# dangvansam/viet-asr

Hardware: AMD Instinct MI355X
Metric: real_time_factor (higher is better)
Workload: dtype f32 via 2xf16 split operands (22-bit significands, 3 f16 MFMA products per multiply, fp32 accumulate); 1 GPU; BASELINE configs[2]: quartznet15x5 greedy CTC, batch=64x10s 16kHz mono per GPU, wav in HBM -> collapsed ids; batch_per_gpu=64, parallelism=utterance-shard x1

## Files before the change

include/vasr_devtools.h:

```cpp
#ifndef VASR_DEVTOOLS_H_
#define VASR_DEVTOOLS_H_
#include "vasr.h"
#ifdef __cplusplus
extern "C" {
#endif

VASR_API int vasr_profile_bracket_overhead(vasr_stream stream, int n, double* out_us);
VASR_API int vasr_fused_tile_choice(int64_t tiles128, int compute_units);
VASR_API int vasr_fused_waves_choice(int kernel, int dual, int tile_cols);
VASR_API int vasr_plan_buffers(vasr_handle* h, int batch, int64_t samples, int64_t mel_frames, int32_t* out, int cap);
VASR_API int vasr_resample_form(double ratio, int nwin, int num_table, int* p, int* q);
VASR_API int vasr_bench_depthwise(const float* d_x, const float* d_w, const int32_t* d_lens, int batch, int channels,
                         int64_t frames, int kernel, float* d_y, vasr_stream stream);
VASR_API int vasr_bench_depthwise_layer(const float* d_x, const float* d_w, const int32_t* d_lens_in, const int32_t* d_lens_out,
                               int batch, int channels, int64_t frames_in, int kernel, int stride, int dilation, float* d_y,
                               uint32_t* d_amax, int amax_stride, vasr_stream stream);
VASR_API int vasr_depthwise_mfma_table_size(int kernel, int dilation);
VASR_API int vasr_pack_depthwise_taps(const float* h_w, int channels, int kernel, int dilation, uint32_t* h_table, float* h_inv);
VASR_API int vasr_bench_depthwise_mfma(const float* d_x, const uint32_t* d_taps, const float* d_tap_inv, const int32_t* d_lens,
                              int batch, int channels, int64_t frames, int kernel, int dilation, float* d_y,
                              uint32_t* d_amax, int amax_stride, vasr_stream stream);
VASR_API int vasr_pack_pointwise(const float* h_w, int cout, int cin, int m_pad, float* h_out);
VASR_API int vasr_conv_gemm_weights(const float* h_w, int cout, int cin, int kernel, float* h_out);
VASR_API int vasr_bench_pointwise(const float* d_x, const float* d_wt, const float* d_scale, const float* d_shift,
                         int batch, int cin, int cout, int64_t frames, float* d_y, vasr_stream stream);

VASR_API int vasr_bench_mfma_sustained(int gemm_mode, int workgroups, int steps, float* d_sink, double* flops, vasr_stream stream);

VASR_API int vasr_pack_pointwise_f16x2(const float* h_w, int cout, int cin, int m_pad, uint16_t* h_out, float* inv_scale);
VASR_API int vasr_bench_pointwise_f16x2(const float* d_x, const uint16_t* d_w16, float w_inv_scale, const float* d_scale,
                               const float* d_shift, int batch, int cin, int cout, int64_t frames, float* d_y,
                               uint32_t* d_amax, int amax_stride, vasr_stream stream);

VASR_API int vasr_pack_pointwise_bf16x3(const float* h_w, int cout, int cin, int m_pad, uint16_t* h_out);
VASR_API int vasr_bench_pointwise_bf16x3(const float* d_x, const uint16_t* d_w3, const float* d_scale, const float* d_shift,
                                int batch, int cin, int cout, int64_t frames, float* d_y, vasr_stream stream);

VASR_API int vasr_bench_groupnorm(const float* d_x, const int32_t* d_lens, int batch, int channels, int64_t frames,
                                  int norm_groups, int shuffle, const float* h_gamma, const float* h_beta, int relu, float* d_y,
                                  vasr_stream stream);
VASR_API int vasr_bench_ctc_head(const float* d_logits, int batch, int64_t frames, int num_classes, float* d_logp,
                                 int64_t* d_pred, vasr_stream stream);
// ... 5 lines not shown
```

viet-asr_amd/_lib.py:

```python
import ctypes as C
import os

import numpy as np
import torch

_HERE = os.path.dirname(os.path.abspath(__file__))
LIB_PATH = os.environ.get("VASR_LIB_PATH") or os.path.join(_HERE, "lib", "libvasr_hip.so")
DEV_LIB_PATH = os.environ.get("VASR_LIB_PATH") or os.path.join(_HERE, "lib", "libvasr_hip_dev.so")


class VasrError(RuntimeError):
    pass


class BlockDesc(C.Structure):
    _fields_ = [(n, C.c_int32) for n in
                ("filters", "repeat", "kernel", "stride", "dilation", "residual", "separable", "residual_dense")]


class FrontendDesc(C.Structure):
    _fields_ = [("sample_rate", C.c_int32), ("n_fft", C.c_int32), ("win_length", C.c_int32),
                ("hop_length", C.c_int32), ("n_mels", C.c_int32), ("preemph", C.c_float),
                ("log_guard", C.c_float), ("normalize", C.c_int32),
                ("h_window", C.POINTER(C.c_float)), ("h_filterbank", C.POINTER(C.c_float)),
# ... 71 lines not shown
    "vasr_classify_f32": (C.c_int, [_P, _P, _P, C.c_int, C.c_int64, C.c_int64, _P, C.c_int, _P, _P, _P, C.c_size_t, _P]),
    "vasr_beam_workspace_bytes": (C.c_size_t, [C.c_int, C.c_int64]),
    "vasr_beam_search_f32": (C.c_int, [_P, C.c_int, C.c_int64, C.c_int, C.c_int, C.c_int, C.c_float, C.c_float, _P,
                                       _P, _P, _P, _P, C.c_size_t, _P]),
    "vasr_beam_search_rows_f32": (C.c_int, [_P, _P, C.c_int, C.c_int64, C.c_int, C.c_int, C.c_int, C.c_float, C.c_float,
                                            _P, _P, _P, _P, _P, C.c_size_t, _P]),
    "vasr_beam_search_nbest_f32": (C.c_int, [_P, _P, C.c_int, C.c_int64, C.c_int, C.c_int, C.c_int, C.c_int, C.c_float,
                                             C.c_float, _P, _P, _P, _P, _P, _P, _P, C.c_size_t, _P]),
    "vasr_lm_create": (C.c_int, [_P, C.c_int, _P, C.c_int, _P, C.c_int, C.c_int, C.c_int, C.c_int, C.c_int, C.c_float,
                                 C.c_float, C.c_float, C.POINTER(_P)]),
    "vasr_lm_destroy": (None, [_P]),
    "vasr_beam_workgroups": (C.c_int, [C.c_int]),
    "vasr_beam_hash_init": (C.c_uint64, []),
    "vasr_beam_hash_step": (C.c_uint64, [C.c_uint64, C.c_uint64]),
    "vasr_last_error": (C.c_char_p, []),
    "vasr_version": (C.c_char_p, []),
    "vasr_abi_version": (C.c_int, []),
    "vasr_algorithmic_work": (C.c_int, [_P, C.c_int, C.c_int64, C.POINTER(C.c_double)]),
    "vasr_profile_begin": (C.c_int, [_P]),
    "vasr_profile_end": (C.c_int, [_P, C.POINTER(C.c_double), C.POINTER(C.c_int64), C.POINTER(C.c_double), C.POINTER(C.c_double)]),
    "vasr_padded_frames": (C.c_int64, [C.c_int64]),
}

DEV_SIGNATURES = {
    "vasr_pack_pointwise_f16x2": (C.c_int, [_P, C.c_int, C.c_int, C.c_int, _P, C.POINTER(C.c_float)]),
    "vasr_bench_pointwise_f16x2": (C.c_int, [_P, _P, C.c_float, _P, _P, C.c_int, C.c_int, C.c_int, C.c_int64, _P, _P,
                                             C.c_int, _P]),
    "vasr_depthwise_mfma_table_size": (C.c_int, [C.c_int, C.c_int]),
    "vasr_pack_depthwise_taps": (C.c_int, [_P, C.c_int, C.c_int, C.c_int, _P, _P]),
    "vasr_bench_depthwise_mfma": (C.c_int, [_P, _P, _P, _P, C.c_int, C.c_int, C.c_int64, C.c_int, C.c_int, _P, _P, C.c_int, _P]),
    "vasr_profile_bracket_overhead": (C.c_int, [_P, C.c_int, C.POINTER(C.c_double)]),
    "vasr_fused_tile_choice": (C.c_int, [C.c_int64, C.c_int]),
    "vasr_fused_waves_choice": (C.c_int, [C.c_int, C.c_int, C.c_int]),
    "vasr_plan_buffers": (C.c_int, [_P, C.c_int, C.c_int64, C.c_int64, C.POINTER(C.c_int32), C.c_int]),
    "vasr_resample_form": (C.c_int, [C.c_double, C.c_int, C.c_int, C.POINTER(C.c_int), C.POINTER(C.c_int)]),
    "vasr_pack_pointwise": (C.c_int, [_P, C.c_int, C.c_int, C.c_int, _P]),
    "vasr_conv_gemm_weights": (C.c_int, [_P, C.c_int, C.c_int, C.c_int, _P]),
    "vasr_pack_pointwise_bf16x3": (C.c_int, [_P, C.c_int, C.c_int, C.c_int, _P]),
    "vasr_bench_pointwise_bf16x3": (C.c_int, [_P, _P, _P, _P, C.c_int, C.c_int, C.c_int, C.c_int64, _P, _P]),
    "vasr_bench_mfma_sustained": (C.c_int, [C.c_int, C.c_int, C.c_int, _P, C.POINTER(C.c_double), _P]),
    "vasr_bench_depthwise": (C.c_int, [_P, _P, _P, C.c_int, C.c_int, C.c_int64, C.c_int, _P, _P]),
    "vasr_bench_depthwise_layer": (C.c_int, [_P, _P, _P, _P, C.c_int, C.c_int, C.c_int64, C.c_int, C.c_int, C.c_int, _P, _P,
                                             C.c_int, _P]),
    "vasr_bench_pointwise": (C.c_int, [_P, _P, _P, _P, C.c_int, C.c_int, C.c_int, C.c_int64, _P, _P]),
    "vasr_bench_groupnorm": (C.c_int, [_P, _P, C.c_int, C.c_int, C.c_int64, C.c_int, C.c_int, _P, _P, C.c_int, _P, _P]),
    "vasr_bench_ctc_head": (C.c_int, [_P, C.c_int, C.c_int64, C.c_int, _P, _P, _P]),
}

ABI_VERSION = 8

_lib = None
_dev = None


def _load(path, tables):
    if not os.path.exists(path):
        raise VasrError(
            f"{path} is missing: build it with `python -c 'import __graft_entry__ as g; g.build()'` "
            "(or `make -C viet-asr_amd/csrc`). There is no CPU fallback for this path.")
    l = C.CDLL(path)
    for table, required in tables:
        for name, (res, args) in table.items():
            fn = getattr(l, name, None)
            if fn is None:
                if required:
                    raise VasrError(f"{path} does not export {name}")
# ... 163 lines not shown
```

viet-asr_amd/csrc/frontend.hip:

```cpp
#include <atomic>

#include "vasr_internal.h"
#include "len_chain.h"
#include "vasr_device.h"

namespace vasr {

namespace {

constexpr int kWaves = 8;
constexpr int kThreads = 64 * kWaves;
constexpr int kNfft = 512;

struct cf { float re, im; };
__device__ __forceinline__ cf cadd(cf a, cf b) { return {a.re + b.re, a.im + b.im}; }
__device__ __forceinline__ cf csub(cf a, cf b) { return {a.re - b.re, a.im - b.im}; }
__device__ __forceinline__ cf cmul(cf a, cf b) { return {a.re * b.re - a.im * b.im, a.re * b.im + a.im * b.re}; }
__device__ __forceinline__ cf cmul_negi(cf a) { return {a.im, -a.re}; }


__device__ __forceinline__ float sample_f32(const float* x, int64_t n) { return x[n]; }
__device__ __forceinline__ float sample_f32(const short* x, int64_t n) { return (float)x[n] * 0x1p-15f; }

template <int kFramesPerBlock, typename S>
// ... 129 lines not shown
  for (int o = 32; o > 0; o >>= 1) v += __shfl_xor(v, o, 64);
  return v;
}

__device__ __forceinline__ int64_t seq_of(int64_t len, int hop) { return (int64_t)ceilf((float)len / (float)hop); }

constexpr int kRowsPerWg = 4;
__device__ __forceinline__ void normalize_row(float* __restrict__ x, int n, int frames, int normalize, double* red) {
  const int tid = threadIdx.x & 255, lane = tid & 63, wv = tid >> 6;
  float mean = 0.f, stdv = 1.f;
  if (normalize) {
    double s = 0.0;
    for (int t = tid; t < n; t += 256) s += (double)x[t];
    s = wave_sum(s);
    if (lane == 0) red[wv] = s;
    __syncthreads();
    const double mu = (((red[0] + red[1]) + red[2]) + red[3]) / (double)n;
    double q = 0.0;
    for (int t = tid; t < n; t += 256) { const double d = (double)x[t] - mu; q += d * d; }
    q = wave_sum(q);
    if (lane == 0) red[4 + wv] = q;
    __syncthreads();
    mean = (float)mu;
    stdv = (float)sqrt((((red[4] + red[5]) + red[6]) + red[7]) / (double)(n - 1));
    stdv = stdv + 1e-5f;
  }
  for (int t = tid; t < frames; t += 256) {
    float v = 0.f;
    if (t < n) v = normalize ? (x[t] - mean) / stdv : x[t];
    x[t] = v;
  }
}

__global__ __launch_bounds__(256 * kRowsPerWg) void normalize_kernel(float* __restrict__ mel, int64_t ld,
                                                                     const int64_t* __restrict__ seq, int rows, int n_mels,
                                                                     int frames, int normalize) {
  __shared__ double red[kRowsPerWg][8];
  const int grp = threadIdx.x >> 8;
  const int row = min((int)blockIdx.x * kRowsPerWg + grp, rows - 1);
  const int64_t n64 = seq[row / n_mels];
  normalize_row(mel + (int64_t)row * ld, (int)(n64 < 0 ? 0 : (n64 > frames ? frames : n64)), frames, normalize, red[grp]);
}

__global__ __launch_bounds__(256) void normalize_all_kernel(float* __restrict__ mel, int64_t ld, const int64_t* __restrict__ seq,
                                                            int n_mels, int frames) {
  __shared__ double red[8];
  const int tid = threadIdx.x, lane = tid & 63, wv = tid >> 6;
  float* x = mel + (int64_t)blockIdx.x * n_mels * ld;
  const int64_t n64 = seq[blockIdx.x];
  const int n = (int)(n64 < 0 ? 0 : (n64 > frames ? frames : n64));
  const double cnt = (double)n * (double)n_mels;
  double s = 0.0;
  for (int f = 0; f < n_mels; ++f)
    for (int t = tid; t < n; t += 256) s += (double)x[(int64_t)f * ld + t];
  s = wave_sum(s);
  if (lane == 0) red[wv] = s;
  __syncthreads();
  const double mu = (((red[0] + red[1]) + red[2]) + red[3]) / cnt;
  double q = 0.0;
  for (int f = 0; f < n_mels; ++f)
    for (int t = tid; t < n; t += 256) { const double d = (double)x[(int64_t)f * ld + t] - mu; q += d * d; }
  q = wave_sum(q);
  if (lane == 0) red[4 + wv] = q;
  __syncthreads();
  const float mean = (float)mu;
  const float stdv = (float)sqrt((((red[4] + red[5]) + red[6]) + red[7]) / (cnt - 1.0)) + 1e-5f;
  for (int f = 0; f < n_mels; ++f)
    for (int t = tid; t < n; t += 256) x[(int64_t)f * ld + t] = (x[(int64_t)f * ld + t] - mean) / stdv;
}

__global__ __launch_bounds__(256 * kRowsPerWg) void normalize_chain_kernel(float* __restrict__ mel, int64_t ld,
                                                              const int64_t* __restrict__ len, int hop, int batch, int n_mels,
                                                              int frames, int normalize, int64_t* __restrict__ seq,
                                                              const LenStep* __restrict__ steps, int n_steps,
                                                              int32_t* __restrict__ lens_tab, float* __restrict__ enc_len,
                                                              const int64_t* __restrict__ wav_len, int frames_cap) {
  __shared__ double red[kRowsPerWg][8];
  const int rows = batch * n_mels, row_wgs = (rows + kRowsPerWg - 1) / kRowsPerWg;
  if ((int)blockIdx.x < row_wgs) {
    const int grp = threadIdx.x >> 8;
    const int row = min((int)blockIdx.x * kRowsPerWg + grp, rows - 1);
    const int64_t n64 = seq_of(len[row / n_mels], hop);
    normalize_row(mel + (int64_t)row * ld, (int)(n64 < 0 ? 0 : (n64 > frames ? frames : n64)), frames, normalize, red[grp]);
    return;
  }
  const int b = ((int)blockIdx.x - row_wgs) * 256 * kRowsPerWg + (int)threadIdx.x;
  const int64_t l0 = b < batch ? seq_of(len[b], hop) : 0;
  if (b < batch) seq[b] = l0;
  len_chain_body(b, l0, batch, steps, n_steps, lens_tab, enc_len, wav_len, hop, frames_cap);
}

}

void launch_stft_logmel(const FrontendTables& tb, const void* wav, bool pcm16, int batch, int64_t samples,
                        const int64_t* row_len, int hop, float preemph, float log_guard, float* mel, int64_t mel_ld, int frames,
                        hipStream_t st) {
  auto go = [&](auto kern, auto* wav, int fpb) {
    const int seg_len = (fpb - 1) * hop + kNfft;
    const size_t lds = (size_t)((seg_len + 3) & ~3) * 4 + kWaves * 256 * 8 + kWaves * (260 + kMelTaps) * 4 + 64 * (fpb + 1) * 4;
    dim3 grid((frames + fpb - 1) / fpb, batch);
    hipLaunchKernelGGL(kern, grid, dim3(kThreads), lds, st, tb, wav, samples, row_len, hop, preemph, log_guard, mel, mel_ld,
                       frames);
  };
  const bool small = (int64_t)((frames + 31) / 32) * batch < 128;
  if (pcm16) {
    if (small) go(stft_logmel_kernel<8, short>, static_cast<const short*>(wav), 8);
    else go(stft_logmel_kernel<32, short>, static_cast<const short*>(wav), 32);
  } else {
    if (small) go(stft_logmel_kernel<8, float>, static_cast<const float*>(wav), 8);
    else go(stft_logmel_kernel<32, float>, static_cast<const float*>(wav), 32);
  }
}

void launch_seq_len(const int64_t* len, int batch, int hop, int64_t* seq, hipStream_t st) {
  hipLaunchKernelGGL(seq_len_kernel, dim3((batch + 63) / 64), dim3(64), 0, st, len, batch, hop, seq);
}

constexpr int kAloneLds = 152 * 1024;

void launch_normalize_all(float* mel, int64_t mel_ld, const int64_t* seq, int batch, int n_mels, int frames, hipStream_t st) {
  static std::atomic<uint64_t> opted{0};
  (void)dyn_lds_opt_in(reinterpret_cast<const void*>(normalize_all_kernel), kAloneLds, opted);
  hipLaunchKernelGGL(normalize_all_kernel, dim3(batch), dim3(256), kAloneLds, st, mel, mel_ld, seq, n_mels, frames);
}

void launch_normalize(float* mel, int64_t mel_ld, const int64_t* seq, int batch, int n_mels, int frames,
                      int normalize, hipStream_t st) {
  const int rows = batch * n_mels;
  static std::atomic<uint64_t> opted{0};
  (void)dyn_lds_opt_in(reinterpret_cast<const void*>(normalize_kernel), kAloneLds, opted);
  hipLaunchKernelGGL(normalize_kernel, dim3((rows + kRowsPerWg - 1) / kRowsPerWg), dim3(256 * kRowsPerWg), normalize ? kAloneLds : 0, st, mel, mel_ld,
                     seq, rows, n_mels, frames, normalize);
}

void launch_normalize_chain(float* mel, int64_t mel_ld, const int64_t* len, int hop, int batch, int n_mels, int frames,
                            int normalize, int64_t* seq, const LenStep* d_steps, int n_steps, int32_t* lens_tab,
                            float* enc_len, const int64_t* wav_len, int frames_cap, hipStream_t st) {
  const int rows = batch * n_mels;
  static std::atomic<uint64_t> opted{0};
  (void)dyn_lds_opt_in(reinterpret_cast<const void*>(normalize_chain_kernel), kAloneLds, opted);
  const int wg = 256 * kRowsPerWg;
  hipLaunchKernelGGL(normalize_chain_kernel, dim3((rows + kRowsPerWg - 1) / kRowsPerWg + (batch + wg - 1) / wg), dim3(wg), normalize ? kAloneLds : 0, st, mel, mel_ld, len, hop, batch,
                     n_mels, frames, normalize, seq, d_steps, n_steps, lens_tab, enc_len, wav_len, frames_cap);
}

}
```

viet-asr_amd/csrc/vasr_api.cpp:

```cpp
#include <hip/hip_runtime.h>

#include <algorithm>
#include <cmath>
#include <cstdarg>
#include <cstdio>
#include <cstring>
#include <memory>
#include <string>

#include "vasr_model.h"

using namespace vasr;

namespace {
thread_local std::string g_err;
}

namespace vasr {

thread_local LaunchProbe g_probe;

int fail(int code, const char* fmt, ...) {
  char buf[512];
  va_list ap;
// ... 173 lines not shown
  if (h->has_encoder && (rc = build_encoder(h))) return rc;
  if (h->has_decoder && (rc = build_decoder(h))) return rc;
  if (h->has_classifier && (rc = build_classifier(h))) return rc;
  HIP_TRY(hipDeviceSynchronize());
  {
    int dev = 0, n = 0;
    if (hipGetDevice(&dev) == hipSuccess && hipDeviceGetAttribute(&n, hipDeviceAttributeMultiprocessorCount, dev) == hipSuccess && n > 0)
      h->n_cu = n;
  }
  h->weights.clear();
  h->finalized = true;
  return 0;
}

int64_t vasr_mel_frames(const vasr_handle* h, int64_t samples) {
  const int hop = (h && h->has_frontend) ? h->fe.hop_length : 160;
  return 1 + samples / hop;
}

int64_t vasr_encoded_frames(const vasr_handle* h, int64_t mel_frames) {
  if (!h || !h->has_encoder || !h->finalized) return mel_frames;
  return enc_frames(h, mel_frames);
}

static size_t sliced_workspace_bytes(const vasr_handle* h, int batch, int64_t T);

static int check_reflect(const vasr_handle* h, int64_t samples) {
  if (samples <= h->fe.n_fft / 2)
    return fail(VASR_ERR_INVALID, "reflect padding needs more than n_fft/2 = %d samples (got %lld)",
                h->fe.n_fft / 2, (long long)samples);
  return 0;
}

static void run_frontend(vasr_handle* h, const float* d_wav, const int64_t* d_len, int batch, int64_t samples, float* mel,
                         int64_t ld, int T, int64_t* seq, hipStream_t st) {
  launch_seq_len(d_len, batch, h->fe.hop_length, seq, st);
  launch_stft_logmel(h->ft, d_wav, false, batch, samples, h->row_independent ? d_len : nullptr, h->fe.hop_length,
                     h->fe.preemph, h->fe.log_guard, mel, ld, T, st);
  launch_normalize(mel, ld, seq, batch, h->fe.n_mels, T, h->fe.normalize == 1, st);
  if (h->fe.normalize == 2) launch_normalize_all(mel, ld, seq, batch, h->fe.n_mels, T, st);
}

size_t vasr_workspace_bytes(const vasr_handle* h, int batch, int64_t samples, int64_t mel_frames) {
  if (!h || !h->finalized || batch <= 0) return 0;
  const int64_t T = samples > 0 ? vasr_mel_frames(h, samples) : mel_frames;
  const size_t whole = plan_ws(h, batch, T).total;
  if (samples > 0 && h->has_frontend && h->has_encoder && h->has_decoder)
    return std::max(whole, sliced_workspace_bytes(h, batch, T));
  return whole;
}

int vasr_melspec_f32(vasr_handle* h, const float* d_wav, const int64_t* d_len, int batch, int64_t samples,
                     float* d_mel, int64_t* d_seq, vasr_stream stream) {
  if (!h || !h->has_frontend || !h->finalized) return fail(VASR_ERR_STATE, "no finalized front end in this handle");
  if (batch <= 0 || !d_wav || !d_len || !d_mel || !d_seq) return fail(VASR_ERR_INVALID, "bad argument");
  if (int rc = check_reflect(h, samples)) return rc;
  hipStream_t st = static_cast<hipStream_t>(stream);
  const int T = (int)vasr_mel_frames(h, samples);
  run_frontend(h, d_wav, d_len, batch, samples, d_mel, T, T, d_seq, st);
  return check_launch("melspec");
}

int vasr_encoder_f32(vasr_handle* h, const float* d_mel, const int64_t* d_seq, int batch, int64_t mel_frames,
                     float* d_enc, float* d_enc_len, void* d_ws, size_t ws_bytes, vasr_stream stream) {
  if (!h || !h->has_encoder || !h->finalized) return fail(VASR_ERR_STATE, "no finalized encoder in this handle");
  if (batch <= 0 || mel_frames <= 0 || !d_mel || !d_seq || !d_enc || !d_ws) return fail(VASR_ERR_INVALID, "bad argument");
  const WsPlan p = plan_ws(h, batch, mel_frames);
  if (ws_bytes < p.total) return fail(VASR_ERR_WORKSPACE, "workspace %zu < %zu bytes", ws_bytes, p.total);
  hipStream_t st = static_cast<hipStream_t>(stream);
  char* ws = static_cast<char*>(d_ws);
  if (port_input_in_place(h))
    return run_encoder(h, d_mel, mel_frames, mel_frames, d_seq, batch, d_enc, p.T1, d_enc_len, ws, p, st);
  float* melp = reinterpret_cast<float*>(ws + p.melp);
  launch_repad(d_mel, mel_frames, batch * h->feat_in, (int)mel_frames, melp, p.Tp0, st);
  return run_encoder(h, melp, p.Tp0, mel_frames, d_seq, batch, d_enc, p.T1, d_enc_len, ws, p, st);
}

int vasr_decoder_logsoftmax_f32(vasr_handle* h, const float* d_enc, int batch, int64_t enc_frames_, float* d_logp,
                                void* d_ws, size_t ws_bytes, vasr_stream stream) {
  if (!h || !h->has_decoder || !h->finalized) return fail(VASR_ERR_STATE, "no finalized decoder in this handle");
  if (batch <= 0 || enc_frames_ <= 0 || !d_enc || !d_logp || !d_ws) return fail(VASR_ERR_INVALID, "bad argument");
  const int64_t ld = pad_frames(enc_frames_);
  const size_t enc_bytes = align_up((size_t)batch * h->dec_feat_in * ld * 4, 256);
  const size_t need_bytes = enc_bytes + (size_t)batch * h->num_classes * ld * 4;
  if (ws_bytes < need_bytes) return fail(VASR_ERR_WORKSPACE, "workspace %zu < %zu bytes", ws_bytes, need_bytes);
  hipStream_t st = static_cast<hipStream_t>(stream);
  float* encp = static_cast<float*>(d_ws);
  float* logits = reinterpret_cast<float*>(static_cast<char*>(d_ws) + enc_bytes);
  launch_repad(d_enc, enc_frames_, batch * h->dec_feat_in, (int)enc_frames_, encp, ld, st);
  AmaxTab ax{};
  const size_t amax_off = align_up(need_bytes, 256), amax_bytes = (size_t)batch * 256 * 4;
  if (h->gemm_mode == 3 && ws_bytes >= amax_off + amax_bytes) {
    ax = AmaxTab{reinterpret_cast<unsigned int*>(static_cast<char*>(d_ws) + amax_off), 256, 0};
    launch_amax(encp, ld, h->dec_feat_in, (int)enc_frames_, nullptr, batch, &ax, st);
  }
  return run_decoder(h, encp, ld, enc_frames_, batch, logits, d_logp, nullptr, st, ax);
}

static int transcribe_part(vasr_handle* h, const void* d_wav, bool pcm16, const int64_t* d_len, int batch, int64_t samples,
                           int64_t* d_pred, int32_t* d_ids, int32_t* d_id_len, float* d_logp, float* d_enc_len,
                           char* ws, hipStream_t st, int row0 = 0) {
  const int64_t T = vasr_mel_frames(h, samples);
  const WsPlan p = plan_ws(h, batch, T);
  int64_t* seq = reinterpret_cast<int64_t*>(ws + p.seq);
  float* melp = reinterpret_cast<float*>(ws + p.melp);
  float* encp = reinterpret_cast<float*>(ws + p.encp);
  float* logits = reinterpret_cast<float*>(ws + p.logits);
  int64_t* pred = d_pred ? d_pred : reinterpret_cast<int64_t*>(ws + p.pred);
  {
    ProfScope ps(h, kProfFrontend, st);
    launch_stft_logmel(h->ft, d_wav, pcm16, batch, samples, h->row_independent ? d_len : nullptr, h->fe.hop_length,
                       h->fe.preemph, h->fe.log_guard, melp, p.Tp0, (int)T, st);
    launch_normalize_chain(melp, p.Tp0, d_len, h->fe.hop_length, batch, h->fe.n_mels, (int)T, h->fe.normalize == 1, seq,
                           h->d_steps, (int)h->steps.size(), reinterpret_cast<int32_t*>(ws + p.lens_tab), d_enc_len,
                           h->row_independent ? d_len : nullptr, (int)p.T1, st);
    if (h->fe.normalize == 2) launch_normalize_all(melp, p.Tp0, seq, batch, h->fe.n_mels, (int)T, st);
  }
  if (h->mask_rects) {
    ProfScope ps(h, kProfFrontend, st);
    launch_spec_mask(melp, p.Tp0, melp, p.Tp0, batch, h->fe.n_mels, (int)T, h->mask_rects, h->mask_row_begin + row0, st);
  }
  AmaxTab enc_amax{};
  const int32_t* own_frames = nullptr;
  int rc = run_encoder(h, melp, p.Tp0, T, seq, batch, encp, p.Tp1, d_enc_len, ws, p, st, &enc_amax, d_len, &own_frames, true);
  if (rc) return rc;
  if ((rc = run_decoder(h, encp, p.Tp1, p.T1, batch, logits, d_logp, pred, st, enc_amax, own_frames))) return rc;
  if (d_ids && d_id_len) {
    ProfScope ps(h, kProfHead, st);
    if (h->row_independent)
      launch_ctc_collapse(pred, batch, p.T1, h->num_classes - 1, d_ids, d_id_len, st, d_len, h->fe.hop_length,
                          h->d_steps, (int)h->steps.size());
    else
      launch_ctc_collapse(pred, batch, p.T1, h->num_classes - 1, d_ids, d_id_len, st);
  }
  return 0;
}

static size_t sliced_workspace_bytes(const vasr_handle* h, int batch, int64_t T) {
  const int n = n_slices(h, batch);
  size_t total = 0;
  for (int i = 0; i < n; ++i) {
    const int lo = slice_bounds(batch, i, n), hi = slice_bounds(batch, i + 1, n);
    total += align_up(plan_ws(h, hi - lo, T).total, 256);
  }
  return total;
}

static int transcribe_any(vasr_handle* h, const void* d_wav, bool pcm16, const int64_t* d_len, int batch, int64_t samples,
                          int64_t* d_pred, int32_t* d_ids, int32_t* d_id_len, float* d_logp, float* d_enc_len,
// ... 94 lines not shown
}
}

size_t vasr_classify_workspace_bytes(const vasr_handle* h, int batch, int64_t samples, int64_t audio_length) {
  if (!h || !h->finalized || !h->has_frontend || !h->has_encoder || !h->has_classifier || batch <= 0 || samples <= 0 ||
      audio_length <= 0)
    return 0;
  return plan_classify(h, batch, samples, audio_length).total;
}

int vasr_classify_f32(vasr_handle* h, const float* d_wav, const int64_t* d_len, int batch, int64_t samples, int64_t audio_length,
                      const int64_t* d_offsets, int softmax, float* d_out, float* d_mel, void* d_ws, size_t ws_bytes,
                      vasr_stream stream) {
  if (!h || !h->finalized || !h->has_frontend || !h->has_encoder || !h->has_classifier)
    return fail(VASR_ERR_STATE, "handle needs a finalized front end, encoder and classifier");
  if (batch <= 0 || !d_wav || !d_len || !d_out || !d_ws || audio_length <= 0 || audio_length > INT32_MAX)
    return fail(VASR_ERR_INVALID, "bad argument");
  if (int rc = check_reflect(h, samples)) return rc;
  if (h->feat_in != h->fe.n_mels) return fail(VASR_ERR_INVALID, "encoder feat_in %d, front end n_mels %d", h->feat_in, h->fe.n_mels);
  const ClsPlan c = plan_classify(h, batch, samples, audio_length);
  if (c.T > audio_length && !d_offsets)
    return fail(VASR_ERR_INVALID, "%lld mel frames are cropped to %lld: offsets needed", (long long)c.T, (long long)audio_length);
  if (ws_bytes < c.total) return fail(VASR_ERR_WORKSPACE, "workspace %zu < %zu bytes", ws_bytes, c.total);
  hipStream_t st = static_cast<hipStream_t>(stream);
  char* ws = static_cast<char*>(d_ws);
  const WsPlan& p = c.enc;
  float* mel_raw = reinterpret_cast<float*>(ws + c.mel_raw);
  int64_t* seq_raw = reinterpret_cast<int64_t*>(ws + c.seq_raw);
  int64_t* seq = reinterpret_cast<int64_t*>(ws + p.seq);
  float* melp = reinterpret_cast<float*>(ws + p.melp);
  float* encp = reinterpret_cast<float*>(ws + p.encp);
  {
    ProfScope ps(h, kProfFrontend, st);
    run_frontend(h, d_wav, d_len, batch, samples, mel_raw, c.Tp, (int)c.T, seq_raw, st);
    const int e = launch_crop_or_pad(mel_raw, c.Tp, batch, h->fe.n_mels, (int)c.T, h->row_independent ? d_len : nullptr,
                                     h->fe.hop_length, (int)audio_length, d_offsets, melp, p.Tp0, (int)p.Tp0, seq, st);
    if (e) return fail(VASR_ERR_HIP, "crop_or_pad: %s", hipGetErrorString((hipError_t)e));
    if (d_mel) launch_repad(melp, p.Tp0, batch * h->fe.n_mels, (int)audio_length, d_mel, audio_length, st);
  }
  int rc = run_encoder(h, melp, p.Tp0, audio_length, seq, batch, encp, p.Tp1, reinterpret_cast<float*>(ws + c.enc_len), ws, p, st);
  if (rc) return rc;
  if ((rc = run_classifier(h, encp, p.Tp1, p.T1, batch, softmax, reinterpret_cast<float*>(ws + c.pooled), d_out, st))) return rc;
  return check_launch("classify");
}

int vasr_set_gemm_mode(vasr_handle* h, int mode) {
  if (!h || mode < 0 || mode > 3)
    return fail(VASR_ERR_INVALID, "gemm mode must be 0 (fp32 MFMA), 1 (3 x bf16 split), 2 (2 x bf16 split, reduced) or "
                                  "3 (2 x fp16 scaled split)");
  h->gemm_mode = mode;
  return 0;
}

int vasr_get_gemm_mode(const vasr_handle* h) { return h ? h->gemm_mode : -1; }

int vasr_set_busy_cus(vasr_handle* h, int cus) {
  if (!h || cus < 0) return fail(VASR_ERR_INVALID, "busy compute units must be >= 0");
  h->busy_cus = cus;
  return 0;
}

int vasr_set_row_independent(vasr_handle* h, int on) {
  if (!h) return fail(VASR_ERR_INVALID, "null handle");
  h->row_independent = on != 0;
  return 0;
}

// ... 72 lines not shown
```

viet-asr_amd/csrc/vasr_devtools.cpp:

```cpp
#include <hip/hip_runtime.h>

#include <algorithm>
#include <cstdio>
#include <cstdlib>
#include <initializer_list>
#include <memory>
#include <string>
#include <vector>

#include "vasr_devtools.h"
#include "vasr_model.h"

using namespace vasr;

const vasr::DevSwitches& vasr::dev_switches() {
  static const DevSwitches sw = [] {
    DevSwitches s;
    auto num = [](const char* name, int dflt, std::initializer_list<int> allowed) {
      const char* e = getenv(name);
      if (!e) return dflt;
      const int v = atoi(e);
      for (int a : allowed) if (a == v) return v;
      fprintf(stderr, "vasr (devtools build): %s=%s is not a documented value -- refusing to guess\n", name, e);
      abort();
      return dflt;
    };
    s.pw3_tile = num("VASR_PW3_TILE", 0, {0, 1, 2, 3, 4, 5});
    s.pw_lat = num("VASR_PW_LAT", 1, {0, 1});
    s.dw_pair = num("VASR_DW_PAIR", 1, {0, 1}) != 0;
    s.dw_mfma = num("VASR_DW_MFMA", 1, {0, 1}) != 0;
    s.dw_upw = num("VASR_DW_UPW", 0, {0, 1, 2, 3, 4, 5, 6, 7, 8});
    s.fused = num("VASR_FUSED", 1, {0, 1}) != 0;
    s.fused_min_tiles = getenv("VASR_FUSED_MIN_TILES") ? atoi(getenv("VASR_FUSED_MIN_TILES")) : 0;
    s.fused_tile = num("VASR_FUSED_TILE", 0, {0, 64, 128});
    s.fused_waves = num("VASR_FUSED_WAVES", 0, {0, 8, 16});
    s.fused_residual = num("VASR_NO_FUSED_RESIDUAL", 0, {0, 1}) == 0;
    s.beam_group = num("VASR_BEAM_GROUP", -1, {-1, 0, 1, 4});
    s.no_grouped = num("VASR_NO_GROUPED", 0, {0, 1}) != 0;
    if (const char* e = getenv("VASR_BUF_ROTATE")) {
      const std::string v(e);
      if (v != "pingpong" && v != "inplace") {
        fprintf(stderr, "vasr (devtools build): VASR_BUF_ROTATE=%s is not a documented value -- refusing to guess\n", e);
        abort();
      }
      s.buf_inplace = v == "inplace";
    }
    return s;
  }();
  return sw;
}

extern "C" {

int vasr_fused_tile_choice(int64_t tiles128, int compute_units) { return vasr::fused_tile_choice(tiles128, compute_units); }
int vasr_fused_waves_choice(int kernel, int dual, int tile_cols) {
  return vasr::fused_waves_choice(kernel, dual != 0, tile_cols, vasr::dev_switches().fused_waves);
}
int vasr_resample_form(double ratio, int nwin, int num_table, int* p, int* q) {
  if (!(ratio > 0.0) || nwin < 2 || num_table < 1 || (int)((ratio < 1.0 ? ratio : 1.0) * num_table) < 1)
    return fail(VASR_ERR_INVALID, "invalid ratio / table for resampling");
  return vasr::resample_form(ratio, nwin, num_table, p, q);
}

static __global__ void dev_noop_kernel() {}

int vasr_profile_bracket_overhead(vasr_stream stream, int n, double* out_us) {
  if (n < 1 || n > 4096 || !out_us) return fail(VASR_ERR_INVALID, "bad argument");
  hipStream_t st = static_cast<hipStream_t>(stream);
  std::vector<hipEvent_t> ev(2 * (size_t)n);
  for (auto& e : ev) HIP_TRY(hipEventCreate(&e));
  for (int i = 0; i < n; ++i) {
    HIP_TRY(hipEventRecord(ev[2 * i], st));
    hipLaunchKernelGGL(dev_noop_kernel, dim3(1), dim3(64), 0, st);
    HIP_TRY(hipEventRecord(ev[2 * i + 1], st));
  }
  HIP_TRY(hipEventSynchronize(ev.back()));
  std::vector<float> t(n);
  for (int i = 0; i < n; ++i) HIP_TRY(hipEventElapsedTime(&t[i], ev[2 * i], ev[2 * i + 1]));
  for (auto& e : ev) (void)hipEventDestroy(e);
  std::sort(t.begin(), t.end());
  *out_us = 1e3 * (double)t[n / 2];
  return 0;
}

int vasr_bench_depthwise(const float* d_x, const float* d_w, const int32_t* d_lens, int batch, int channels,
                         int64_t frames, int kernel, float* d_y, vasr_stream stream) {
  if (!d_x || !d_w || !d_lens || !d_y) return fail(VASR_ERR_INVALID, "bad argument");
  const int64_t ld = pad_frames(frames);
  (void)launch_depthwise(d_x, ld, (int)frames, d_w, d_lens, d_lens, batch, channels, kernel, 1, 1, kernel / 2, d_y, ld,
// ... 226 lines not shown
```

viet-asr_amd/csrc/vasr_internal.h:

```cpp
#pragma once
#include <hip/hip_runtime.h>
#include <atomic>
#include <hip/hip_ext.h>
#include <stdint.h>
#include <stdlib.h>

namespace vasr {

struct DevSwitches {
  int pw3_tile = 0;
  int pw_lat = 1;
  bool dw_pair = true;
  bool dw_mfma = true;
  int dw_upw = 0;
  bool fused = true;
  int fused_min_tiles = 0;
  int fused_tile = 0;
  int fused_waves = 0;
  bool fused_residual = true;
  int beam_group = -1;
  bool no_grouped = false;
  bool buf_inplace = true;
};
#ifdef VASR_DEVTOOLS
const DevSwitches& dev_switches();
#else
inline const DevSwitches& dev_switches() { static constexpr DevSwitches k{}; return k; }
#endif

struct LaunchProbe { hipEvent_t start = nullptr, stop = nullptr; };
extern thread_local LaunchProbe g_probe;
#define VASR_LAUNCH(kern, grid, block, lds, st, ...)                                                       \
  do {                                                                                                     \
    if (::vasr::g_probe.start) {                                                                           \
      hipExtLaunchKernelGGL(kern, grid, block, lds, st, ::vasr::g_probe.start, ::vasr::g_probe.stop, 0,   \
                            __VA_ARGS__);                                                                  \
      ::vasr::g_probe.start = nullptr;                                                                     \
    } else {                                                                                               \
      hipLaunchKernelGGL(kern, grid, block, lds, st, __VA_ARGS__);                                         \
    }                                                                                                      \
  } while (0)

inline hipError_t dyn_lds_opt_in(const void* kernel, int bytes, std::atomic<uint64_t>& done) {
  int dev = 0;
  if (hipGetDevice(&dev) != hipSuccess) dev = 0;
  const uint64_t bit = 1ull << (dev & 63);
  if (done.load(std::memory_order_relaxed) & bit) return hipSuccess;
  const hipError_t e = hipFuncSetAttribute(kernel, hipFuncAttributeMaxDynamicSharedMemorySize, bytes);
  if (e == hipSuccess) done.fetch_or(bit, std::memory_order_relaxed);
  return e;
}

#define VASR_LAUNCH_PART(first, last, kern, grid, block, lds, st, ...)                                     \
  do {                                                                                                     \
    if (::vasr::g_probe.start) {                                                                           \
      hipExtLaunchKernelGGL(kern, grid, block, lds, st, (first) ? ::vasr::g_probe.start : nullptr,         \
                            (last) ? ::vasr::g_probe.stop : nullptr, 0, __VA_ARGS__);                      \
      if (last) ::vasr::g_probe.start = nullptr;                                                           \
    } else {                                                                                               \
      hipLaunchKernelGGL(kern, grid, block, lds, st, __VA_ARGS__);                                         \
    }                                                                                                      \
  } while (0)

constexpr int kTimeTile = 128;
static inline int64_t pad_frames(int64_t t) { return (t + kTimeTile - 1) / kTimeTile * kTimeTile; }


struct AmaxTab {
  unsigned int* p = nullptr;
  int stride = 0;
  int n = 0;
};

struct FrontendTables {
  const float* window;
  const float* tw256;
  const float* tw512;
  const float* mel_w;
  const int32_t* mel_lo;
  int32_t guard_clamp;
};
constexpr int kMelTaps = 32;

void launch_stft_logmel(const FrontendTables& tb, const void* wav, bool pcm16, int batch, int64_t samples,
                        const int64_t* row_len, int hop, float preemph, float log_guard, float* mel, int64_t mel_ld, int frames,
                        hipStream_t st);
void launch_seq_len(const int64_t* len, int batch, int hop, int64_t* seq, hipStream_t st);
void launch_normalize_all(float* mel, int64_t mel_ld, const int64_t* seq, int batch, int n_mels, int frames, hipStream_t st);
void launch_normalize(float* mel, int64_t mel_ld, const int64_t* seq, int batch, int n_mels, int frames,
                      int normalize, hipStream_t st);

struct LenStep { int32_t kernel, stride, dilation, pad; };
void launch_normalize_chain(float* mel, int64_t mel_ld, const int64_t* len, int hop, int batch, int n_mels, int frames,
                            int normalize, int64_t* seq, const LenStep* d_steps, int n_steps, int32_t* lens_tab,
                            float* enc_len, const int64_t* wav_len, int frames_cap, hipStream_t st);
void launch_len_chain(const int64_t* seq, int batch, const LenStep* d_steps, int n_steps, int32_t* lens_tab,
                      float* enc_len, hipStream_t st, const int64_t* wav_len = nullptr, int hop = 1, int frames_cap = 0);

void launch_repad(const float* src, int64_t src_ld, int rows, int frames, float* dst, int64_t dst_ld,
                  hipStream_t st);

int launch_depthwise(const float* x, int64_t ldx, int frames_in, const float* w, const int32_t* lens_in,
                     const int32_t* lens_out, int batch, int channels, int kernel, int stride, int dilation,
                     int pad, float* y, int64_t ldy, hipStream_t st, AmaxTab* amax_y = nullptr);
int depthwise_amax_slots(int channels, int64_t ldy);

int depthwise_mfma_table_size(int kernel, int dilation);
float pack_depthwise_taps_f16x2(const float* w, int kernel, int dilation, int tsz, unsigned int* table);
int launch_depthwise_mfma(const float* x, int64_t ldx, const unsigned int* taps, const float* tap_inv,
                          const int32_t* lens_in, const int32_t* lens_out, AmaxTab amax_x, int batch,
                          int channels, int kernel, int dilation, float* y, int64_t ldy, AmaxTab* amax_y,
                          hipStream_t st);

enum : int32_t { kActRelu = 0, kActHardtanh = 1, kActSelu = 2 };

inline int epilogue_kind(int relu, int act, bool res_max) {
  if ((relu & 1) && act == kActSelu) return 2;
  return (((relu & 1) && act != kActRelu) || res_max) ? 1 : 0;
}

struct PwArgs {
  const float* wt;
  const float* x;
  const int32_t* lens;
  const float* x2;
  const int32_t* lens2;
  int32_t K1;
  int64_t ldx2;
// ... 233 lines not shown
```

Before: 126,400 audio-sec/wall-sec.

## Hold mel rows in registers and prefetch next row in persistent normalize kernel

The per-feature normalization kernels become grid-strided over rows, sized to the compute-unit count. A templated held path keeps the first 1024 frames of each row in registers and prefetches the next row while the current one is reduced and written. This aims to cut repeated global reads of each row across the mean, variance and write passes, and to hide load latency. In exchange it adds register pressure and a fallback loop for longer rows, plus error propagation when the LDS opt-in is refused.

Measured after the change: 126,500 audio-sec/wall-sec, median of 6. Within noise of the previous version (+0.1%).

```diff
diff --git a/include/vasr_devtools.h b/include/vasr_devtools.h
--- a/include/vasr_devtools.h
+++ b/include/vasr_devtools.h
@@ -8,6 +8,7 @@
 VASR_API int vasr_profile_bracket_overhead(vasr_stream stream, int n, double* out_us);
 VASR_API int vasr_fused_tile_choice(int64_t tiles128, int compute_units);
 VASR_API int vasr_fused_waves_choice(int kernel, int dual, int tile_cols);
+VASR_API int vasr_dev_switch(const char* name);
 VASR_API int vasr_plan_buffers(vasr_handle* h, int batch, int64_t samples, int64_t mel_frames, int32_t* out, int cap);
 VASR_API int vasr_resample_form(double ratio, int nwin, int num_table, int* p, int* q);
 VASR_API int vasr_bench_depthwise(const float* d_x, const float* d_w, const int32_t* d_lens, int batch, int channels,
diff --git a/viet-asr_amd/_lib.py b/viet-asr_amd/_lib.py
--- a/viet-asr_amd/_lib.py
+++ b/viet-asr_amd/_lib.py
@@ -127,6 +127,7 @@
     "vasr_profile_bracket_overhead": (C.c_int, [_P, C.c_int, C.POINTER(C.c_double)]),
     "vasr_fused_tile_choice": (C.c_int, [C.c_int64, C.c_int]),
     "vasr_fused_waves_choice": (C.c_int, [C.c_int, C.c_int, C.c_int]),
+    "vasr_dev_switch": (C.c_int, [C.c_char_p]),
     "vasr_plan_buffers": (C.c_int, [_P, C.c_int, C.c_int64, C.c_int64, C.POINTER(C.c_int32), C.c_int]),
     "vasr_resample_form": (C.c_int, [C.c_double, C.c_int, C.c_int, C.POINTER(C.c_int), C.POINTER(C.c_int)]),
     "vasr_pack_pointwise": (C.c_int, [_P, C.c_int, C.c_int, C.c_int, _P]),
diff --git a/viet-asr_amd/csrc/frontend.hip b/viet-asr_amd/csrc/frontend.hip
--- a/viet-asr_amd/csrc/frontend.hip
+++ b/viet-asr_amd/csrc/frontend.hip
@@ -185,14 +185,82 @@
   }
 }
 
+constexpr int kHeld = 4;
+__device__ __forceinline__ void held_load(const float* __restrict__ x, int frames, float (&v)[kHeld]) {
+  const int tid = threadIdx.x & 255;
+#pragma unroll
+  for (int j = 0; j < kHeld; ++j) v[j] = x[min(tid + 256 * j, frames - 1)];
+}
+__device__ __forceinline__ void held_finish(float* __restrict__ x, int n, int frames, int normalize, double* red,
+                                            const float (&v)[kHeld]) {
+  const int tid = threadIdx.x & 255, lane = tid & 63, wv = tid >> 6;
+  float mean = 0.f, stdv = 1.f;
+  if (normalize) {
+    double s = 0.0;
+#pragma unroll
+    for (int j = 0; j < kHeld; ++j) if (tid + 256 * j < n) s += (double)v[j];
+    for (int t = tid + 256 * kHeld; t < n; t += 256) s += (double)x[t];
+    s = wave_sum(s);
+    if (lane == 0) red[wv] = s;
+    __syncthreads();
+    const double mu = (((red[0] + red[1]) + red[2]) + red[3]) / (double)n;
+    double q = 0.0;
+#pragma unroll
+    for (int j = 0; j < kHeld; ++j) if (tid + 256 * j < n) { const double d = (double)v[j] - mu; q += d * d; }
+    for (int t = tid + 256 * kHeld; t < n; t += 256) { const double d = (double)x[t] - mu; q += d * d; }
+    q = wave_sum(q);
+    if (lane == 0) red[4 + wv] = q;
+    __syncthreads();
+    mean = (float)mu;
+    stdv = (float)sqrt((((red[4] + red[5]) + red[6]) + red[7]) / (double)(n - 1));
+    stdv = stdv + 1e-5f;
+  }
+#pragma unroll
+  for (int j = 0; j < kHeld; ++j) {
+    const int t = tid + 256 * j;
+    if (t < frames) x[t] = t < n ? (normalize ? (v[j] - mean) / stdv : v[j]) : 0.f;
+  }
+  for (int t = tid + 256 * kHeld; t < frames; t += 256) {
+    float w = 0.f;
+    if (t < n) w = normalize ? (x[t] - mean) / stdv : x[t];
+    x[t] = w;
+  }
+}
+
+template <bool HELD, class LenOf>
+__device__ __forceinline__ void normalize_rows(float* __restrict__ mel, int64_t ld, int rows, int n_mels, int frames,
+                                               int normalize, double* red, int q0, int step, int quads, LenOf len_of) {
+  const int grp = threadIdx.x >> 8;
+  auto row_of = [&](int q) { return min(q * kRowsPerWg + grp, rows - 1); };
+  auto n_of = [&](int row) {
+    const int64_t n64 = len_of(row / n_mels);
+    return (int)(n64 < 0 ? 0 : (n64 > frames ? frames : n64));
+  };
+  if constexpr (HELD) {
+    float v[kHeld], vn[kHeld];
+    if (q0 < quads) held_load(mel + (int64_t)row_of(q0) * ld, frames, v);
+    for (int q = q0; q < quads; q += step) {
+      const int row = row_of(q), qn = q + step < quads ? q + step : q;
+      held_load(mel + (int64_t)row_of(qn) * ld, frames, vn);
+      held_finish(mel + (int64_t)row * ld, n_of(row), frames, normalize, red, v);
+#pragma unroll
+      for (int j = 0; j < kHeld; ++j) v[j] = vn[j];
+    }
+  } else {
+    for (int q = q0; q < quads; q += step) {
+      const int row = row_of(q);
+      normalize_row(mel + (int64_t)row * ld, n_of(row), frames, normalize, red);
+    }
+  }
+}
+
+template <bool HELD>
 __global__ __launch_bounds__(256 * kRowsPerWg) void normalize_kernel(float* __restrict__ mel, int64_t ld,
                                                                      const int64_t* __restrict__ seq, int rows, int n_mels,
                                                                      int frames, int normalize) {
   __shared__ double red[kRowsPerWg][8];
-  const int grp = threadIdx.x >> 8;
-  const int row = min((int)blockIdx.x * kRowsPerWg + grp, rows - 1);
-  const int64_t n64 = seq[row / n_mels];
-  normalize_row(mel + (int64_t)row * ld, (int)(n64 < 0 ? 0 : (n64 > frames ? frames : n64)), frames, normalize, red[grp]);
+  normalize_rows<HELD>(mel, ld, rows, n_mels, frames, normalize, red[threadIdx.x >> 8], (int)blockIdx.x, (int)gridDim.x,
+                       (rows + kRowsPerWg - 1) / kRowsPerWg, [&](int b) { return seq[b]; });
 }
 
 __global__ __launch_bounds__(256) void normalize_all_kernel(float* __restrict__ mel, int64_t ld, const int64_t* __restrict__ seq,
@@ -222,19 +290,18 @@
     for (int t = tid; t < n; t += 256) x[(int64_t)f * ld + t] = (x[(int64_t)f * ld + t] - mean) / stdv;
 }
 
+template <bool HELD>
 __global__ __launch_bounds__(256 * kRowsPerWg) void normalize_chain_kernel(float* __restrict__ mel, int64_t ld,
                                                               const int64_t* __restrict__ len, int hop, int batch, int n_mels,
                                                               int frames, int normalize, int64_t* __restrict__ seq,
                                                               const LenStep* __restrict__ steps, int n_steps,
                                                               int32_t* __restrict__ lens_tab, float* __restrict__ enc_len,
-                                                              const int64_t* __restrict__ wav_len, int frames_cap) {
+                                                              const int64_t* __restrict__ wav_len, int frames_cap, int row_wgs) {
   __shared__ double red[kRowsPerWg][8];
-  const int rows = batch * n_mels, row_wgs = (rows + kRowsPerWg - 1) / kRowsPerWg;
   if ((int)blockIdx.x < row_wgs) {
-    const int grp = threadIdx.x >> 8;
-    const int row = min((int)blockIdx.x * kRowsPerWg + grp, rows - 1);
-    const int64_t n64 = seq_of(len[row / n_mels], hop);
-    normalize_row(mel + (int64_t)row * ld, (int)(n64 < 0 ? 0 : (n64 > frames ? frames : n64)), frames, normalize, red[grp]);
+    const int rows = batch * n_mels;
+    normalize_rows<HELD>(mel, ld, rows, n_mels, frames, normalize, red[threadIdx.x >> 8], (int)blockIdx.x, row_wgs,
+                         (rows + kRowsPerWg - 1) / kRowsPerWg, [&](int b) { return seq_of(len[b], hop); });
     return;
   }
   const int b = ((int)blockIdx.x - row_wgs) * 256 * kRowsPerWg + (int)threadIdx.x;
@@ -271,30 +338,56 @@
 
 constexpr int kAloneLds = 152 * 1024;
 
-void launch_normalize_all(float* mel, int64_t mel_ld, const int64_t* seq, int batch, int n_mels, int frames, hipStream_t st) {
+int launch_normalize_all(float* mel, int64_t mel_ld, const int64_t* seq, int batch, int n_mels, int frames, hipStream_t st) {
   static std::atomic<uint64_t> opted{0};
-  (void)dyn_lds_opt_in(reinterpret_cast<const void*>(normalize_all_kernel), kAloneLds, opted);
+  const hipError_t attr = dyn_lds_opt_in(reinterpret_cast<const void*>(normalize_all_kernel), kAloneLds, opted);
+  if (attr != hipSuccess) return (int)attr;
   hipLaunchKernelGGL(normalize_all_kernel, dim3(batch), dim3(256), kAloneLds, st, mel, mel_ld, seq, n_mels, frames);
-}
-
-void launch_normalize(float* mel, int64_t mel_ld, const int64_t* seq, int batch, int n_mels, int frames,
-                      int normalize, hipStream_t st) {
+  return 0;
+}
+
+static int row_workgroups(int quads) {
+  static std::atomic<int> units[64];
+  int dev = 0;
+  if (hipGetDevice(&dev) != hipSuccess) dev = 0;
+  int cu = units[dev & 63].load(std::memory_order_relaxed);
+  if (cu <= 0) {
+    if (hipDeviceGetAttribute(&cu, hipDeviceAttributeMultiprocessorCount, dev) != hipSuccess || cu <= 0) cu = 256;
+    units[dev & 63].store(cu, std::memory_order_relaxed);
+  }
+  const int trips = (quads + cu - 1) / cu;
+  return trips ? (quads + trips - 1) / trips : 1;
+}
+
+int launch_normalize(float* mel, int64_t mel_ld, const int64_t* seq, int batch, int n_mels, int frames,
+                     int normalize, hipStream_t st) {
   const int rows = batch * n_mels;
-  static std::atomic<uint64_t> opted{0};
-  (void)dyn_lds_opt_in(reinterpret_cast<const void*>(normalize_kernel), kAloneLds, opted);
-  hipLaunchKernelGGL(normalize_kernel, dim3((rows + kRowsPerWg - 1) / kRowsPerWg), dim3(256 * kRowsPerWg), normalize ? kAloneLds : 0, st, mel, mel_ld,
-                     seq, rows, n_mels, frames, normalize);
-}
-
-void launch_normalize_chain(float* mel, int64_t mel_ld, const int64_t* len, int hop, int batch, int n_mels, int frames,
-                            int normalize, int64_t* seq, const LenStep* d_steps, int n_steps, int32_t* lens_tab,
-                            float* enc_len, const int64_t* wav_len, int frames_cap, hipStream_t st) {
+  auto go = [&](auto kern, std::atomic<uint64_t>& opted) {
+    const hipError_t attr = dyn_lds_opt_in(reinterpret_cast<const void*>(kern), kAloneLds, opted);
+    if (attr != hipSuccess) return (int)attr;
+    hipLaunchKernelGGL(kern, dim3(row_workgroups((rows + kRowsPerWg - 1) / kRowsPerWg)), dim3(256 * kRowsPerWg), normalize ? kAloneLds : 0, st, mel, mel_ld,
+                       seq, rows, n_mels, frames, normalize);
+    return 0;
+  };
+  static std::atomic<uint64_t> opted[2];
+  return dev_switches().norm_held ? go(normalize_kernel<true>, opted[1]) : go(normalize_kernel<false>, opted[0]);
+}
+
+int launch_normalize_chain(float* mel, int64_t mel_ld, const int64_t* len, int hop, int batch, int n_mels, int frames,
+                           int normalize, int64_t* seq, const LenStep* d_steps, int n_steps, int32_t* lens_tab,
+                           float* enc_len, const int64_t* wav_len, int frames_cap, hipStream_t st) {
   const int rows = batch * n_mels;
-  static std::atomic<uint64_t> opted{0};
-  (void)dyn_lds_opt_in(reinterpret_cast<const void*>(normalize_chain_kernel), kAloneLds, opted);
   const int wg = 256 * kRowsPerWg;
-  hipLaunchKernelGGL(normalize_chain_kernel, dim3((rows + kRowsPerWg - 1) / kRowsPerWg + (batch + wg - 1) / wg), dim3(wg), normalize ? kAloneLds : 0, st, mel, mel_ld, len, hop, batch,
-                     n_mels, frames, normalize, seq, d_steps, n_steps, lens_tab, enc_len, wav_len, frames_cap);
-}
-
-}
+  const int row_wgs = row_workgroups((rows + kRowsPerWg - 1) / kRowsPerWg);
+  auto go = [&](auto kern, std::atomic<uint64_t>& opted) {
+    const hipError_t attr = dyn_lds_opt_in(reinterpret_cast<const void*>(kern), kAloneLds, opted);
+    if (attr != hipSuccess) return (int)attr;
+    hipLaunchKernelGGL(kern, dim3(row_wgs + (batch + wg - 1) / wg), dim3(wg), normalize ? kAloneLds : 0, st, mel, mel_ld, len, hop, batch,
+                       n_mels, frames, normalize, seq, d_steps, n_steps, lens_tab, enc_len, wav_len, frames_cap, row_wgs);
+    return 0;
+  };
+  static std::atomic<uint64_t> opted[2];
+  return dev_switches().norm_held ? go(normalize_chain_kernel<true>, opted[1]) : go(normalize_chain_kernel<false>, opted[0]);
+}
+
+}
diff --git a/viet-asr_amd/csrc/vasr_api.cpp b/viet-asr_amd/csrc/vasr_api.cpp
--- a/viet-asr_amd/csrc/vasr_api.cpp
+++ b/viet-asr_amd/csrc/vasr_api.cpp
@@ -229,13 +229,18 @@
   return 0;
 }
 
-static void run_frontend(vasr_handle* h, const float* d_wav, const int64_t* d_len, int batch, int64_t samples, float* mel,
+static int norm_rc(int e) {
+  return e ? fail(VASR_ERR_HIP, "normalisation: the opt-in for its dynamic LDS was refused: %s", hipGetErrorString((hipError_t)e)) : 0;
+}
+
+static int run_frontend(vasr_handle* h, const float* d_wav, const int64_t* d_len, int batch, int64_t samples, float* mel,
                          int64_t ld, int T, int64_t* seq, hipStream_t st) {
   launch_seq_len(d_len, batch, h->fe.hop_length, seq, st);
   launch_stft_logmel(h->ft, d_wav, false, batch, samples, h->row_independent ? d_len : nullptr, h->fe.hop_length,
                      h->fe.preemph, h->fe.log_guard, mel, ld, T, st);
-  launch_normalize(mel, ld, seq, batch, h->fe.n_mels, T, h->fe.normalize == 1, st);
-  if (h->fe.normalize == 2) launch_normalize_all(mel, ld, seq, batch, h->fe.n_mels, T, st);
+  if (int rc = norm_rc(launch_normalize(mel, ld, seq, batch, h->fe.n_mels, T, h->fe.normalize == 1, st))) return rc;
+  if (h->fe.normalize == 2) return norm_rc(launch_normalize_all(mel, ld, seq, batch, h->fe.n_mels, T, st));
+  return 0;
 }
 
 size_t vasr_workspace_bytes(const vasr_handle* h, int batch, int64_t samples, int64_t mel_frames) {
@@ -254,7 +259,7 @@
   if (int rc = check_reflect(h, samples)) return rc;
   hipStream_t st = static_cast<hipStream_t>(stream);
   const int T = (int)vasr_mel_frames(h, samples);
-  run_frontend(h, d_wav, d_len, batch, samples, d_mel, T, T, d_seq, st);
+  if (int rc = run_frontend(h, d_wav, d_len, batch, samples, d_mel, T, T, d_seq, st)) return rc;
   return check_launch("melspec");
 }
 
@@ -308,10 +313,11 @@
     ProfScope ps(h, kProfFrontend, st);
     launch_stft_logmel(h->ft, d_wav, pcm16, batch, samples, h->row_independent ? d_len : nullptr, h->fe.hop_length,
                        h->fe.preemph, h->fe.log_guard, melp, p.Tp0, (int)T, st);
-    launch_normalize_chain(melp, p.Tp0, d_len, h->fe.hop_length, batch, h->fe.n_mels, (int)T, h->fe.normalize == 1, seq,
-                           h->d_steps, (int)h->steps.size(), reinterpret_cast<int32_t*>(ws + p.lens_tab), d_enc_len,
-                           h->row_independent ? d_len : nullptr, (int)p.T1, st);
-    if (h->fe.normalize == 2) launch_normalize_all(melp, p.Tp0, seq, batch, h->fe.n_mels, (int)T, st);
+    int rc = norm_rc(launch_normalize_chain(melp, p.Tp0, d_len, h->fe.hop_length, batch, h->fe.n_mels, (int)T, h->fe.normalize == 1,
+                                            seq, h->d_steps, (int)h->steps.size(), reinterpret_cast<int32_t*>(ws + p.lens_tab),
+                                            d_enc_len, h->row_independent ? d_len : nullptr, (int)p.T1, st));
+    if (!rc && h->fe.normalize == 2) rc = norm_rc(launch_normalize_all(melp, p.Tp0, seq, batch, h->fe.n_mels, (int)T, st));
+    if (rc) return rc;
   }
   if (h->mask_rects) {
     ProfScope ps(h, kProfFrontend, st);
@@ -472,7 +478,7 @@
   float* encp = reinterpret_cast<float*>(ws + p.encp);
   {
     ProfScope ps(h, kProfFrontend, st);
-    run_frontend(h, d_wav, d_len, batch, samples, mel_raw, c.Tp, (int)c.T, seq_raw, st);
+    if (int rc = run_frontend(h, d_wav, d_len, batch, samples, mel_raw, c.Tp, (int)c.T, seq_raw, st)) return rc;
     const int e = launch_crop_or_pad(mel_raw, c.Tp, batch, h->fe.n_mels, (int)c.T, h->row_independent ? d_len : nullptr,
                                      h->fe.hop_length, (int)audio_length, d_offsets, melp, p.Tp0, (int)p.Tp0, seq, st);
     if (e) return fail(VASR_ERR_HIP, "crop_or_pad: %s", hipGetErrorString((hipError_t)e));
diff --git a/viet-asr_amd/csrc/vasr_devtools.cpp b/viet-asr_amd/csrc/vasr_devtools.cpp
--- a/viet-asr_amd/csrc/vasr_devtools.cpp
+++ b/viet-asr_amd/csrc/vasr_devtools.cpp
@@ -37,6 +37,7 @@
     s.fused_residual = num("VASR_NO_FUSED_RESIDUAL", 0, {0, 1}) == 0;
     s.beam_group = num("VASR_BEAM_GROUP", -1, {-1, 0, 1, 4});
     s.no_grouped = num("VASR_NO_GROUPED", 0, {0, 1}) != 0;
+    s.norm_held = num("VASR_NORM_HELD", 1, {0, 1}) != 0;
     if (const char* e = getenv("VASR_BUF_ROTATE")) {
       const std::string v(e);
       if (v != "pingpong" && v != "inplace") {
@@ -55,6 +56,11 @@
 int vasr_fused_tile_choice(int64_t tiles128, int compute_units) { return vasr::fused_tile_choice(tiles128, compute_units); }
 int vasr_fused_waves_choice(int kernel, int dual, int tile_cols) {
   return vasr::fused_waves_choice(kernel, dual != 0, tile_cols, vasr::dev_switches().fused_waves);
+}
+int vasr_dev_switch(const char* name) {
+  const std::string n(name ? name : "");
+  if (n == "norm_held") return vasr::dev_switches().norm_held ? 1 : 0;
+  return fail(VASR_ERR_INVALID, "vasr_dev_switch: no switch named '%s'", n.c_str());
 }
 int vasr_resample_form(double ratio, int nwin, int num_table, int* p, int* q) {
   if (!(ratio > 0.0) || nwin < 2 || num_table < 1 || (int)((ratio < 1.0 ? ratio : 1.0) * num_table) < 1)
diff --git a/viet-asr_amd/csrc/vasr_internal.h b/viet-asr_amd/csrc/vasr_internal.h
--- a/viet-asr_amd/csrc/vasr_internal.h
+++ b/viet-asr_amd/csrc/vasr_internal.h
@@ -21,6 +21,7 @@
   int beam_group = -1;
   bool no_grouped = false;
   bool buf_inplace = true;
+  bool norm_held = true;
 };
 #ifdef VASR_DEVTOOLS
 const DevSwitches& dev_switches();
@@ -86,14 +87,14 @@
                         const int64_t* row_len, int hop, float preemph, float log_guard, float* mel, int64_t mel_ld, int frames,
                         hipStream_t st);
 void launch_seq_len(const int64_t* len, int batch, int hop, int64_t* seq, hipStream_t st);
-void launch_normalize_all(float* mel, int64_t mel_ld, const int64_t* seq, int batch, int n_mels, int frames, hipStream_t st);
-void launch_normalize(float* mel, int64_t mel_ld, const int64_t* seq, int batch, int n_mels, int frames,
-                      int normalize, hipStream_t st);
+int launch_normalize_all(float* mel, int64_t mel_ld, const int64_t* seq, int batch, int n_mels, int frames, hipStream_t st);
+int launch_normalize(float* mel, int64_t mel_ld, const int64_t* seq, int batch, int n_mels, int frames,
+                     int normalize, hipStream_t st);
 
 struct LenStep { int32_t kernel, stride, dilation, pad; };
-void launch_normalize_chain(float* mel, int64_t mel_ld, const int64_t* len, int hop, int batch, int n_mels, int frames,
-                            int normalize, int64_t* seq, const LenStep* d_steps, int n_steps, int32_t* lens_tab,
-                            float* enc_len, const int64_t* wav_len, int frames_cap, hipStream_t st);
+int launch_normalize_chain(float* mel, int64_t mel_ld, const int64_t* len, int hop, int batch, int n_mels, int frames,
+                           int normalize, int64_t* seq, const LenStep* d_steps, int n_steps, int32_t* lens_tab,
+                           float* enc_len, const int64_t* wav_len, int frames_cap, hipStream_t st);
 void launch_len_chain(const int64_t* seq, int batch, const LenStep* d_steps, int n_steps, int32_t* lens_tab,
                       float* enc_len, hipStream_t st, const int64_t* wav_len = nullptr, int hop = 1, int frames_cap = 0);
 
```
